# speechcatcher-asr/speechcatcher

Measured on AMD Instinct MI355X. Metric: concurrent real-time streams (audio-seconds/s), de_xl dims, 640 ms (10240-sample) chunk steps, beam 10 CTC+attention, higher is better.
Workload: dtype f32

## Files before the change

### speechcatcher_amd/csrc/common.h

```cpp
#pragma once
#include <hip/hip_runtime.h>
#include <stdint.h>
#include <stdio.h>
#include <math.h>

#include "../../include/scasr.h"

#define SC_LOGZERO (-10000000000.0f)

void sc_set_error(const char *fmt, ...);

const char *sc_hook(const char *name);

#define SC_CHECK_ARG(cond, msg)      \
  do {                               \
    if (!(cond)) {                   \
      sc_set_error("%s: %s", __func__, msg); \
      return SC_ERR_ARG;             \
    }                                \
  } while (0)

#define SC_CHECK_LAUNCH()                                              \
  do {                                                                 \
    hipError_t e__ = hipGetLastError();                                \
    if (e__ != hipSuccess) {                                           \
      sc_set_error("%s: launch failed: %s", __func__, hipGetErrorString(e__)); \
      return SC_ERR_LAUNCH;                                            \
    }                                                                  \
  } while (0)

__host__ __device__ static inline int cdiv(int a, int b) { return (a + b - 1) / b; }

struct ProfScope { bool on; hipEvent_t a, b; hipStream_t st; };
ProfScope sc_prof_begin(hipStream_t st);
void sc_prof_end(ProfScope &p, int kind, double flops, double bytes);

int sc_decode_step_form(const sc_search *sb);
int sc_gemm_colblocks(const float *A, const int32_t *a_rows, int lda, const float *W, const float *bias, float *C,
                      const int32_t *c_rows, int ldc, int M, int N, int K, int ncb, long cb_stride, int flags, void *stream);

int sc_dec_layer_hpw(const sc_search &sb);
int sc_dec_layer_stream_form(const sc_search &sb);
int sc_dec_layer_split_ffn(const sc_search &sb);

int sc_launch_reduce_ln_proj(const float *part, int npart, int part_M, const float *b2, const float *Xin, float *Xout,
                             const int32_t *rows, int M, int D, const float *ln_g, const float *ln_b, float ln_eps,
                             float *XN, const float *Wq, const float *bq, float *Q, int N, hipStream_t st,
                             int by_row = 0, int half_mode = 0);

struct ScHandoff { const int32_t *blkinfo; int R; float *state; int layer; };
int sc_ffn_ln_handoff(const float *XN, int M, int D, int F, const void *W1, const float *b1, const void *W2, const float *b2,
                      float *X, int w_form, const ScHandoff &ho, void *stream);

template <int CTRL>
__device__ __forceinline__ float dpp_mov(float v) {
  return __int_as_float(__builtin_amdgcn_update_dpp(0, __float_as_int(v), CTRL, 0xF, 0xF, true));
}
#define SC_DPP_XOR1 0xB1
#define SC_DPP_XOR2 0x4E
#define SC_DPP_HALF_MIRROR 0x141
#define SC_DPP_ROR4 0x124
#define SC_DPP_ROR8 0x128
#define SC_DPP_ROW_MIRROR 0x140

template <int LPR>
__device__ __forceinline__ float group_sum(float v) {
  v += dpp_mov<SC_DPP_XOR1>(v);
  v += dpp_mov<SC_DPP_XOR2>(v);
  if (LPR >= 8) v += dpp_mov<SC_DPP_HALF_MIRROR>(v);
  if (LPR == 16) v += dpp_mov<SC_DPP_ROW_MIRROR>(v);
  return v;
}

__device__ __forceinline__ float sc_lane(float v, int lane) {
  return __int_as_float(__builtin_amdgcn_readlane(__float_as_int(v), lane));
}
__device__ __forceinline__ float wave_max(float v) {
  v = fmaxf(v, dpp_mov<SC_DPP_XOR1>(v));
  v = fmaxf(v, dpp_mov<SC_DPP_XOR2>(v));
  v = fmaxf(v, dpp_mov<SC_DPP_HALF_MIRROR>(v));
  v = fmaxf(v, dpp_mov<SC_DPP_ROW_MIRROR>(v));
  return fmaxf(fmaxf(sc_lane(v, 0), sc_lane(v, 16)), fmaxf(sc_lane(v, 32), sc_lane(v, 48)));
}
__device__ __forceinline__ float wave_sum(float v) {
  v += dpp_mov<SC_DPP_XOR1>(v);
  v += dpp_mov<SC_DPP_XOR2>(v);
  v += dpp_mov<SC_DPP_HALF_MIRROR>(v);
  v += dpp_mov<SC_DPP_ROW_MIRROR>(v);
  return (sc_lane(v, 0) + sc_lane(v, 16)) + (sc_lane(v, 32) + sc_lane(v, 48));
}
// ... 93 lines not shown
```

### speechcatcher_amd/csrc/search.hip

```cpp
#include "common.h"
#include "attn.h"
#include <mutex>
#include <unordered_map>

#define CTRL(s, f) sb.ctrl[(s) * 8 + (f)]
#define SC_CTC_T(s) (CTRL(s, SC_C_TCTC) > 0 ? CTRL(s, SC_C_TCTC) : CTRL(s, SC_C_T))

#define YSEQ(pp, s, h) (sb.yseq + (((long)(pp) * sb.S + (s)) * sb.W + (h)) * sb.LCAP)
#define XPOS(pp, s, h) (sb.xpos + (((long)(pp) * sb.S + (s)) * sb.W + (h)) * sb.LCAP)
#define ANC(pp, s) (sb.anc + ((long)(pp) * sb.S + (s)) * sb.LCAP * sb.W)
#define CTCR(pp, s) (sb.ctc_r + ((long)(pp) * sb.S + (s)) * sb.TCAP * 2 * sb.W)
#define CTCRS(pp, s) (sb.ctc_rs + ((long)(pp) * sb.S + (s)) * sb.TCAP * sb.W)

__global__ void ctc_extend_state_kernel(sc_search sb) {
  const int s = blockIdx.x, h = threadIdx.x;
  if (!CTRL(s, SC_C_ACTIVE) || !CTRL(s, SC_C_HAS)) return;
  const int T = CTRL(s, SC_C_T), told = CTRL(s, SC_C_TOLD), nh = CTRL(s, SC_C_NHYP);
  if (h >= nh || told >= T) return;
  float *r = CTCR(CTRL(s, SC_C_CUR), s);
  float *rs = CTCRS(CTRL(s, SC_C_CUR), s);
  const float *x = sb.ctcx + (long)s * sb.TCAP * sb.V;
  const int t0 = told < 1 ? 1 : told;
  float rb = r[((long)(t0 - 1) * 2 + 1) * sb.W + h];
  for (int t = t0; t < T; ++t) {
// ... 862 lines not shown
      const bool ok = kw != 0ull && sort_key_value(kw) > bound;
      if (lane == 0) need_full = ok ? 0 : 1;
      if (ok && lane < W) {
        const int i = sort_key_index(key);
        sb.cand_tok[(long)row * W + lane] = i;
        sb.cand_score[(long)row * W + lane] = sort_key_value(key);
        sb.cand_ctc[(long)row * W + lane] = ctc[i];
      }
    }
    __syncthreads();
    if (!need_full) return;
    __syncthreads();
  }
  for (int v = tid; v < V; v += 256) ctc[v] = SC_LOGZERO;
  __syncthreads();
  for (int k = tid; k < K; k += 256) ctc[sb.pre_ids[(long)row * K + k]] = sb.psi[(long)row * K + k];
  __syncthreads();
  if (tid == 0) {
    ctc[sb.eos] = sb.psi_eos[row];
    ctc[sb.blank] = SC_LOGZERO;
  }
  __syncthreads();
  for (int v = tid; v < V; v += 256) {
    const float cv = __fsub_rn(ctc[v], s_prev);
    ctc[v] = cv;
    comb[v] = __fadd_rn(__fmul_rn(sb.w_dec, sb.logp[(long)row * V + v]), __fmul_rn(sb.w_ctc, cv));
  }
  __syncthreads();
  const int NP = next_pow2(V);
  unsigned long long *comp = reinterpret_cast<unsigned long long *>(smem + 2 * V);
  for (int c = tid; c < NP; c += 256) comp[c] = c < V ? sort_key(comb[c], c) : 0ull;
  __syncthreads();
  block_bitonic_sort_desc(comp, NP);
  for (int k = tid; k < W; k += 256) {
    const int i = sort_key_index(comp[k]);
    sb.cand_tok[(long)row * W + k] = i;
    sb.cand_score[(long)row * W + k] = comb[i];
    sb.cand_ctc[(long)row * W + k] = ctc[i];
  }
}

extern "C" int sc_fuse_topw(const sc_search *sbp, void *stream) {
  SC_CHECK_ARG(sbp, "null");
  SC_CHECK_ARG(sbp->V > 0 && sbp->V <= SC_MAX_VOCAB, "vocabulary larger than SC_MAX_VOCAB (8192)");
  const size_t smem = fuse_topw_lds(sbp->V);
  const int rc = allow_large_lds(reinterpret_cast<const void *>(&fuse_topw_kernel), smem, fuse_topw_lds(SC_MAX_VOCAB),
                                 "sc_fuse_topw");
  if (rc != SC_OK) return rc;
  fuse_topw_kernel<<<sbp->S * sbp->W, 256, smem, (hipStream_t)stream>>>(*sbp);
  SC_CHECK_LAUNCH();
  return SC_OK;
}

__global__ __launch_bounds__(256) void beam_prune_kernel(sc_search sb) {
  extern __shared__ __attribute__((aligned(16))) double tot[];
  __shared__ int fl_any, fl_all, fl_best, fl_rep;
  __shared__ int win_h[64], win_tok[64];
  __shared__ unsigned bm[SC_KV_MAX_ROWS / 32];
  const int s = blockIdx.x, tid = threadIdx.x;
  if (!CTRL(s, SC_C_ACTIVE)) return;
  for (int w = tid; w < (sb.kv_rows + 31) / 32; w += 256) bm[w] = 0u;
  const int W = sb.W, K = sb.K;
  const int nh = CTRL(s, SC_C_NHYP), L = CTRL(s, SC_C_L), T = CTRL(s, SC_C_T);
  const int cur = CTRL(s, SC_C_CUR), o = 1 - cur;
  const int n = nh * W, nout = n < W ? n : W;
  if (tid == 0) { fl_any = 0; fl_all = 1; fl_best = 0; fl_rep = 0; }
  for (int e = tid; e < n; e += 256) {
    const int h = e / W, j = e % W;
    tot[e] = sb.score[((long)cur * sb.S + s) * W + h] + (double)sb.cand_score[((long)s * W + h) * W + j];
  }
  __syncthreads();
  for (int e = tid; e < n; e += 256) {
    const double te = tot[e];
    int rk = 0;
    for (int j = 0; j < n; ++j) rk += (tot[j] > te) || (tot[j] == te && j < e);
    if (rk >= nout) continue;
    const int h = e / W, j = e % W, i = rk;
    const long prow = (long)s * W + h;
    const int tok = sb.cand_tok[prow * W + j];
    win_h[i] = h;
    win_tok[i] = tok;
    const long oi = ((long)o * sb.S + s) * W + i, ci = ((long)cur * sb.S + s) * W + h;
    sb.score[oi] = te;
    sb.sc_dec[oi] = sb.sc_dec[ci] + (double)sb.logp[prow * sb.V + tok];
    sb.sc_ctc[oi] = sb.sc_ctc[ci] + (double)sb.cand_ctc[prow * W + j];
    int kk = -1;
    for (int q = 0; q < K; ++q)
      if (sb.pre_ids[prow * K + q] == tok) { kk = q; break; }
    float sval;
    if (tok == sb.blank) sval = SC_LOGZERO;
    else if (tok == sb.eos) sval = sb.psi_eos[prow];
    else if (kk >= 0) sval = sb.psi[prow * K + kk];
    else sval = SC_LOGZERO;
    sb.ctc_s[oi] = sval;
    sb.sel[((long)s * W + i) * 2] = h;
    sb.sel[((long)s * W + i) * 2 + 1] = kk < 0 ? 0 : kk;
    const bool is_eos = tok == sb.eos;
    if (is_eos) atomicOr(&fl_any, 1);
    else atomicAnd(&fl_all, 0);
    if (i == 0 && is_eos) atomicOr(&fl_best, 1);
  }
  __syncthreads();
  const int *asrc = ANC(cur, s);
  int *adst = ANC(o, s);
  bool rep = false;
  constexpr int UB = 4;
  const int ntot = nout * (L + 1);
// ... 9 lines not shown
      av[u] = asrc[(long)p * W + h];
    }
#pragma unroll
    for (int u = 0; u < UB; ++u) {
      const int e = e0 + 256 * u;
      if (e >= ntot) break;
      const int i = e / (L + 1), p = e % (L + 1);
      const int tok = win_tok[i];
      int *ydst = YSEQ(o, s, i), *xdst = XPOS(o, s, i);
      if (p < L) {
        ydst[p] = yv[u];
        xdst[p] = xv[u];
        if (p >= 1 && yv[u] == tok && tok != sb.sos && tok != sb.eos) rep = true;
        adst[(long)p * W + i] = av[u];
        atomicOr(&bm[(av[u] >> 5) & (SC_KV_MAX_ROWS / 32 - 1)], 1u << (av[u] & 31));
      } else {
        ydst[L] = tok;
        xdst[L] = T - 1;
      }
    }
  }
  if (rep) atomicOr(&fl_rep, 1);
  __syncthreads();
  if (tid == 0)
    sb.flags[s] = (fl_any ? SC_F_ANY_EOS : 0) | (fl_best ? SC_F_BEST_EOS : 0) |
                  (fl_all ? SC_F_ALL_EOS : 0) | (fl_rep ? SC_F_REPEAT : 0);
  if (tid >= 64 || L + 1 > sb.LCAP) return;
  const int lane = tid, NR = sb.kv_rows, nwords = (NR + 31) / 32;
  int *out = adst + (long)L * W;
  int got = 0;
  for (int w0 = 0; w0 < nwords && got < nout; w0 += 64) {
    const int w = w0 + lane;
    unsigned fr = w < nwords ? ~bm[w] : 0u;
    if (w == nwords - 1 && (NR & 31)) fr &= (1u << (NR & 31)) - 1u;
    const int c = __popc(fr);
    int incl = c;
#pragma unroll
    for (int o2 = 1; o2 < 64; o2 <<= 1) {
      const int t = __shfl_up(incl, o2, 64);
      if (lane >= o2) incl += t;
    }
    int k = got + incl - c;
    while (fr && k < nout) {
      const int b = __ffs(fr) - 1;
      fr &= fr - 1u;
      out[k++] = w * 32 + b;
    }
    got += __shfl(incl, 63, 64);
  }
  if (got < nout && lane >= got && lane < nout) out[lane] = NR - 1;
  if (lane == 0 && sb.kvflags) sb.kvflags[s] = got < nout ? 1 : 0;
}

extern "C" int sc_beam_prune(const sc_search *sbp, void *stream) {
  SC_CHECK_ARG(sbp, "null");
  SC_CHECK_ARG(sbp->W <= 64, "beam wider than 64");
  SC_CHECK_ARG(sbp->kv_rows >= sbp->W && sbp->kv_rows <= SC_KV_MAX_ROWS, "kv_rows out of range (beam .. 65536)");
  size_t smem = (size_t)sbp->W * sbp->W * sizeof(double);
  beam_prune_kernel<<<sbp->S, 256, smem, (hipStream_t)stream>>>(*sbp);
  SC_CHECK_LAUNCH();
  return SC_OK;
}

__global__ __launch_bounds__(256) void ctc_gather_state_kernel(sc_search sb, int split_min) {
  const int s = blockIdx.y;
  if (!CTRL(s, SC_C_ACTIVE)) return;
  const int W = sb.W, K = sb.K, V = sb.V, T = SC_CTC_T(s), nh = CTRL(s, SC_C_NHYP), L = CTRL(s, SC_C_L);
  const int nout = nh * W < W ? nh * W : W;
  const int cur = CTRL(s, SC_C_CUR), o = 1 - cur;
  const bool has = CTRL(s, SC_C_HAS);
  const int WK = W * K, tct = sb.tct;
  float *dst = CTCR(o, s);
  float *dst_rs = CTCRS(o, s);
  const float *__restrict__ rp = CTCR(cur, s);
  const float *__restrict__ rsp = CTCRS(cur, s);
  const float *ck = sb.ctc_rnew + (long)s * ctc_tck(sb.TCAP) * 2 * WK;
  const int out_len = L - 1;
  int start = out_len > 1 ? out_len : 1;
  if (start > T) start = T;
  const bool split = ctc_scan_is_split(T, L, split_min);
  const int base = start & ~15;
  const int seg = split ? 16 * cdiv(T - base, 16 * CTC_NSEG) : SC_CTC_CK;
  const int nseg = split ? CTC_NSEG : cdiv(T, SC_CTC_CK);
  for (int idx = blockIdx.x * blockDim.x + threadIdx.x; idx < nout * nseg; idx += gridDim.x * blockDim.x) {
    const int i = idx % nout, j = idx / nout;
    const int h = sb.sel[((long)s * W + i) * 2], k = sb.sel[((long)s * W + i) * 2 + 1];
    const int e = h * K + k;
    const int c = sb.pre_ids[((long)s * W + h) * K + k];
    const bool same = c == YSEQ(cur, s, h)[L - 1];
    const float *__restrict__ xcol = sb.ctcxT + ((long)s * V + c) * tct;
    const float *__restrict__ xblk = sb.ctcxT + ((long)s * V + sb.blank) * tct;
    int t_lo, t_hi;
    float r_n, r_b;
    if (split) {
      t_lo = max(start, base + j * seg);
      t_hi = min(T, base + (j + 1) * seg);
      r_n = ck[((long)j * 2) * WK + e];
      r_b = ck[((long)j * 2 + 1) * WK + e];
      if (j == 0) {
        for (int t = 0; t < start - 1; ++t) {
          dst[((long)t * 2) * W + i] = SC_LOGZERO;
          dst[((long)t * 2 + 1) * W + i] = SC_LOGZERO;
          dst_rs[(long)t * W + i] = lse2(SC_LOGZERO, SC_LOGZERO);
        }
        dst[((long)(start - 1) * 2) * W + i] = (out_len == 0) ? xcol[0] : SC_LOGZERO;
        dst[((long)(start - 1) * 2 + 1) * W + i] = SC_LOGZERO;
        dst_rs[(long)(start - 1) * W + i] = lse2((out_len == 0) ? xcol[0] : SC_LOGZERO, SC_LOGZERO);
      }
    } else {
      const int t0 = j * SC_CTC_CK, t1 = min(t0 + SC_CTC_CK, T);
      if (t0 <= start - 1) {
        r_n = (out_len == 0) ? xcol[0] : SC_LOGZERO;
        r_b = SC_LOGZERO;
        for (int t = t0; t < min(start - 1, t1); ++t) {
          dst[((long)t * 2) * W + i] = SC_LOGZERO;
// ... 30 lines not shown
      for (int q = 0; q < SC_CTC_CK; ++q) {
        const int tp = min(max(tb + q - 1, 0), T - 1);
        pn[q] = has ? rsp[(long)tp * W + h] : 0.f;
        pb[q] = has ? rp[((long)tp * 2 + 1) * W + h] : 0.f;
      }
#pragma unroll
      for (int q = 0; q < SC_CTC_CK; ++q) {
        const int t = tb + q;
        if (t >= t_lo && t < t_hi) {
          float phi;
          ctc_frame(r_n, r_b, has ? pn[q] : cum, has ? pb[q] : cum, same, xc[q], xb[q], phi);
          dst[((long)t * 2) * W + i] = r_n;
          dst[((long)t * 2 + 1) * W + i] = r_b;
          dst_rs[(long)t * W + i] = lse2(r_n, r_b);
          if (!has) cum += xb[q];
        }
      }
    }
  }
}

extern "C" int sc_ctc_gather_state_split(const sc_search *sbp, int split_min, void *stream) {
  SC_CHECK_ARG(sbp, "null");
  SC_CHECK_ARG(sbp->ctcxT && sbp->tct >= 4, "the state rebuild needs the column-major table copy (sc_search.ctcxT)");
  int gx = cdiv(ctc_tck(sbp->TCAP) * sbp->W, 256);
  if (gx > 16) gx = 16;
  const int eff = ctc_split_min_ok(sbp->TCAP, split_min), last = scan_split_last(sbp);
  if (last >= 0 && last != eff) {
    sc_set_error("sc_ctc_gather_state_split: the last prefix scan of this batch ran with split_min = %d, the rebuild was asked for %d - "
                 "streams split over T leave segment states, not checkpoints: pass the scan's value (sc_ctc_gather_state() = 0)", last, eff);
    return SC_ERR_ARG;
  }
  ctc_gather_state_kernel<<<dim3(gx, sbp->S), 256, 0, (hipStream_t)stream>>>(*sbp, eff);
  SC_CHECK_LAUNCH();
  return SC_OK;
}

extern "C" int sc_ctc_gather_state(const sc_search *sbp, void *stream) { return sc_ctc_gather_state_split(sbp, 0, stream); }

static bool dec_fused_ok(const sc_search &sb) {
  if (const char *e = sc_hook("SC_DEC_FUSED"))
    return atoi(e) != 0 && sc_dec_layer_fused_supported(sb.d, sb.H, sb.W, sb.F) && sb.ph1 && sb.out_w_q;
  if (const char *e = sc_hook("SC_FUSED_MAX"))
    if ((sb.rowmap ? sb.n_rows : sb.S * sb.W) > atoi(e) && sc_dec_layer_hpw(sb) < 2) return false;
  return sc_dec_layer_fused_supported(sb.d, sb.H, sb.W, sb.F) && sb.ph1 && sb.ph2 && sb.ffn_part &&
         sb.max_ffn_part >= 1 && sb.out_w_q && sb.V % sb.d == 0 && sb.layers && sb.layers[0].wqkv_pp &&
         sb.layers[0].wq_pp && sb.layers[0].wo_pp && sb.layers[0].w1_p;
}

int sc_decode_step_form(const sc_search *sbp) { return dec_fused_ok(*sbp) ? (sc_dec_layer_stream_form(*sbp) ? 2 : 1) : 0; }

extern "C" int sc_decode_step(const sc_search *sbp, void *stream) { return sc_decode_step_ex(sbp, 0, stream); }

extern "C" int sc_decode_step_ex(const sc_search *sbp, int scan_split_min, void *stream) {
  SC_CHECK_ARG(sbp, "null");
  const sc_search &sb = *sbp;
  const int n = sb.rowmap ? sb.n_rows : sb.S * sb.W;
  int rc;
  if (dec_fused_ok(sb) && sc_dec_layer_stream_form(sb)) {
    float *xa = sb.dx, *xb = sb.dxn;
    int npart = 0;
    for (int li = 0; li < sb.n_layers; ++li) {
      SC_TRY(sc_dec_layer_stream(sbp, li, xa, xb, sb.dq, sb.ffn_part, npart, stream));
      SC_TRY(sc_dec_layer_ffn_xn(sbp, li, sb.dq, sb.ffn_part, sb.max_ffn_part, &npart, stream));
      float *t = xa; xa = xb; xb = t;
    }
    SC_TRY(sc_dec_output_logits(sbp, xa, xb, sb.ffn_part, npart, stream));
  } else if (dec_fused_ok(sb)) {
    float *xa = sb.dx, *xb = sb.dxn;
    int npart = 0;
    for (int li = 0; li < sb.n_layers; ++li) {
      SC_TRY(sc_dec_layer_self(sbp, li, xa, xb, sb.ffn_part, npart, stream));
      SC_TRY(sc_dec_layer_cross(sbp, li, xb, xa, stream));
      if (sc_dec_layer_split_ffn(sb)) {
        SC_TRY(sc_dec_layer_reduce_ln(sbp, li, xa, xb, sb.dq, stream));
        SC_TRY(sc_dec_layer_ffn_xn(sbp, li, sb.dq, sb.ffn_part, sb.max_ffn_part, &npart, stream));
      } else
      SC_TRY(sc_dec_layer_ffn(sbp, li, xa, xb, sb.ffn_part, sb.max_ffn_part, &npart, stream));
      float *t = xa; xa = xb; xb = t;
    }
    SC_TRY(sc_dec_output_logits(sbp, xa, xb, sb.ffn_part, npart, stream));
  } else {
  SC_TRY(sc_dec_embed(sbp, stream));
  bool logits_done = false;
  SC_TRY(decoder_layers_impl(sbp, stream, true, &logits_done));
  if (!logits_done)
    SC_TRY(sc_gemm(sb.dxn, sb.rowmap, sb.d, sb.out_w, sb.out_b, sb.logits, sb.rowmap, sb.V, n, sb.V, sb.d, 0, 0, stream));
  }
  SC_TRY(sc_logsoftmax_topk(sbp, stream));
  const bool use_ctc = sb.w_ctc > 0.f;
  if (use_ctc) SC_TRY(sc_ctc_prefix_scan_split(sbp, scan_split_min, stream));
  SC_TRY(sc_fuse_topw(sbp, stream));
  SC_TRY(sc_beam_prune(sbp, stream));
  if (use_ctc) SC_TRY(sc_ctc_gather_state_split(sbp, scan_split_min, stream));
  return SC_OK;
}
```

### speechcatcher_amd/csrc/streams.hip

```cpp
#include <algorithm>
#include <array>
#include <chrono>
#include <cmath>
#include <cstdarg>
#include <cstring>
#include <deque>
#include <map>
#include <memory>
#include <new>
#include <string>
#include <vector>

#include "common.h"

namespace {

#define HIP_TRY(call)                                                              \
  do {                                                                             \
    hipError_t e__ = (call);                                                       \
    if (e__ != hipSuccess) {                                                       \
      sc_set_error("%s: %s failed: %s", __func__, #call, hipGetErrorString(e__));  \
      return SC_ERR_LAUNCH;                                                        \
    }                                                                              \
  } while (0)
#define RC_TRY(call)                 \
  do {                               \
    int rc__ = (call);               \
    if (rc__ != SC_OK) return rc__;  \
  } while (0)

struct Tensor {
  void *ptr = nullptr;
  int64_t numel = 0;
  int dtype = 0;
  bool owned = false;
};

struct StreamFault {
  int stream;
  int code;
  std::string msg;
};

}

struct sc_engine {
  sc_config cfg{};
  int device = 0;
  std::map<std::string, Tensor> t;
  std::vector<sc_enc_layer> enc;
  std::vector<sc_dec_layer> dec;
  std::vector<const float *> wkv, bkv;
  float *wkv_all = nullptr, *bkv_all = nullptr;

  const float *f(const std::string &name, bool required = true) const {
    auto it = t.find(name);
    if (it == t.end()) {
      if (required) sc_set_error("sc_engine: tensor '%s' is missing", name.c_str());
      return nullptr;
    }
    return (const float *)it->second.ptr;
  }
  ~sc_engine() {
    for (auto &kv : t)
      if (kv.second.owned && kv.second.ptr) (void)hipFree(kv.second.ptr);
    if (wkv_all) (void)hipFree(wkv_all);
// ... 49 lines not shown
};

template <typename T>
int dalloc(T **p, size_t n) {
  const size_t bytes = std::max<size_t>(n, 1) * sizeof(T);
  HIP_TRY(hipMalloc((void **)p, bytes));
  HIP_TRY(hipMemset(*p, 0, bytes));
  return SC_OK;
}

}

struct EncPlan {
  std::vector<int32_t> conv_jobs, a_rows, lin_dst, feat_src, feat_dst, blk_jobs, sjobs, emit_src, emit_dst, sub_src,
      sub_dst;
  struct Short { int s, ubase, U, pe_pos, dst_T; };
  std::vector<Short> shorts;
  int n_conv = 0, max_t1 = 0;
};

struct EncGroup {
  long gen = 0;
  bool launched = false, features = false;
  bool open = false;
  bool deferred = false;
  int slot = 0;
  int stage_slot = -1;
  std::vector<long long> copy_jobs;
  size_t stage_floats = 0;
  std::vector<int32_t> fe_jobs;
  int n_fe = 0, max_keep = 0;
  EncPlan P;
  std::vector<int32_t> ctc_rows, kv_src, kv_dst;
  bool same_rows = true;
  std::vector<int> streams;
  bool empty() const { return !n_fe && !P.n_conv; }
};

constexpr int N_ARENA = 8;
constexpr int N_STAGE = 4;
constexpr int N_RING = 4;

struct sc_streams {
  sc_engine *eng = nullptr;
  sc_config cfg{};
  int S = 0, W = 0, K = 0, TCAP = 0, LCAP = 0, FCAP = 0, UCAP = 0, max_feat_new = 0, max_t1 = 0, max_t2 = 0,
      max_blocks = 0, max_chunk = 0, max_length = 500;
  long PCAP = 0;
  bool use_bbd = false, strict = true;
  hipStream_t stream = nullptr;
  hipStream_t stream_enc = nullptr, es = nullptr;
  hipEvent_t ev_iter[2] = {nullptr, nullptr};
  int32_t *ring_dev = nullptr;
  int32_t *rm_host[2] = {nullptr, nullptr};
  int rm_idx = 0;
  bool rm_dirty = false;
  int scan_split_min = 1024, scan_split_streams = 0;
  bool scan_long = false;
  int step_split_min() const { return (scan_long && (scan_split_streams <= 0 || n_rows_step <= scan_split_streams * W)) ? scan_split_min : 0; }
  int graph_key() const { return n_rows_step * 2 + (step_split_min() > 0 ? 1 : 0); }
  int enc_start_thr = 0;
  int enc_batch_min = 0;
  int gemm_flags = 0;
  void *ws = nullptr, *ws_enc = nullptr;
  std::vector<void *> owned, owned_host;
  float *pcm = nullptr, *featbuf = nullptr, *subbuf = nullptr, *prev_addin = nullptr, *past_ctx = nullptr, *enc = nullptr,
        *c1 = nullptr, *c2 = nullptr, *xblk = nullptr, *ws_xn = nullptr, *ws_qkv = nullptr, *ws_att = nullptr,
        *ws_ffh = nullptr;
  int32_t *jobs_ctx = nullptr, *ctrlmap = nullptr;
  float *kv_stage = nullptr;
  int kv_stage_rows = 0;
  sc_search sb{};
  int32_t *ctrlmap_host = nullptr, *flags_host = nullptr;
  int32_t *arena_host = nullptr, *arena_dev = nullptr;
  size_t slot_cap = 0, arena_off = 0;
  int cur_slot = 0;
  hipEvent_t ev_group[N_ARENA] = {nullptr};
  long slot_gen[N_ARENA] = {0};
  int32_t *bs_host = nullptr, *bs_dev = nullptr;
  size_t bs_cap = 0;
  int bs_i = 0;
  float *stage_host = nullptr, *stage_dev = nullptr;
  size_t stage_cap = 0;
  hipEvent_t ev_stage[N_STAGE] = {nullptr};
  bool stage_busy[N_STAGE] = {false};
  int stage_next = 0;
  long long *cjobs_host = nullptr, *cjobs_dev = nullptr;
  int32_t *pack_dev = nullptr, *pack_host = nullptr, *pjobs_host = nullptr, *pjobs_dev = nullptr;
  size_t pack_cap = 0;
  char *al_dev = nullptr;
  size_t al_cap = 0;
  std::vector<St> st;
  std::vector<Run> run;
  std::vector<std::deque<Blk>> bq;
  std::vector<Job> job;
  std::vector<std::deque<Job>> ahead;
  std::vector<long> job_seq;
  int queue_depth = 1;
  std::vector<Snap> snap;
  std::vector<long> done_at;
  long done_counter = 0;
  int32_t *snap_yseq = nullptr, *snap_xpos = nullptr;
  double *snap_score = nullptr;
  hipEvent_t ev_snap = nullptr;
  std::vector<std::string> fault_msg;
  std::vector<long> enc_gen;
// ... 419 lines not shown
    std::vector<int32_t> j_add(ns * 4), j_ctx(ns * 4);
    for (int i = 0; i < ns; ++i) {
      const int32_t *sj = &P.sjobs[i * 5];
      j_add[i * 4 + 0] = sj[0]; j_add[i * 4 + 1] = sj[1]; j_add[i * 4 + 2] = sj[2]; j_add[i * 4 + 3] = sj[3];
      j_ctx[i * 4 + 0] = sj[0]; j_ctx[i * 4 + 1] = sj[1]; j_ctx[i * 4 + 2] = sj[2] * c.enc_layers; j_ctx[i * 4 + 3] = sj[4];
    }
    RC_TRY(b->itensor(j_add, &ja));
    RC_TRY(sc_ctx_handoff(b->xblk, R, ja, ns, b->prev_addin, 0, d, b->es));
    const int32_t *jc;
    RC_TRY(b->itensor(j_ctx, &jc));
    HIP_TRY(hipMemcpyAsync(b->jobs_ctx, jc, j_ctx.size() * sizeof(int32_t), hipMemcpyDeviceToDevice, b->es));
    RC_TRY(enc_layers_launch(b, nbk, R, true, b->jobs_ctx, ns));
  }
  if (!P.emit_src.empty()) {
    const int32_t *a, *z;
    RC_TRY(b->itensor(P.emit_src, &a));
    RC_TRY(b->itensor(P.emit_dst, &z));
    RC_TRY(sc_layernorm(b->xblk, a, d, b->enc, z, d, (int)P.emit_src.size(), d, e->f("enc_norm_g"), e->f("enc_norm_b"),
                        c.ln_eps, b->es));
  }
  for (auto &sh : P.shorts) RC_TRY(encode_short(b, sh));
  if (!P.sub_src.empty()) {
    const int32_t *a, *z;
    RC_TRY(b->itensor(P.sub_src, &a));
    RC_TRY(b->itensor(P.sub_dst, &z));
    RC_TRY(sc_copy_rows(b->subbuf, a, b->subbuf, z, (int)P.sub_src.size(), d, b->es));
  }
  return SC_OK;
}

void set_rowmap(sc_streams *b, const std::vector<int> &active) {
  const int S = b->S, W = b->W;
  const int na = (int)active.size();
  const int nb = std::min(S, (na + b->row_bucket - 1) / b->row_bucket * b->row_bucket);
  if (active != b->rowmap_key) {
    b->rowmap_key = active;
    b->rm_idx ^= 1;
    b->rm_dirty = true;
    int32_t *rm = b->rowmap_host();
    std::vector<char> isact(S, 0);
    for (int s : active) isact[s] = 1;
    int k = 0;
    for (int pass = 1; pass >= 0; --pass)
      for (int s = 0; s < S; ++s)
        if (isact[s] == pass)
          for (int h = 0; h < W; ++h) rm[k++] = s * W + h;
  }
  b->n_rows_step = nb * W;
}

int decode_step_launch(sc_streams *b) {
  b->sb.n_rows = b->n_rows_step;
  b->sb.flags = b->ring_dev;
  auto step = [&]() { return sc_decode_step_ex(&b->sb, b->step_split_min(), b->stream); };
  if (!b->use_graphs) return step();
  auto it = b->dec_graphs.find(b->graph_key());
  if (it == b->dec_graphs.end()) {
    RC_TRY(step());
    RC_TRY(sc_graph_capture_begin(b->stream));
    const int rc = step();
    void *g = nullptr;
    const int rc2 = sc_graph_capture_end(b->stream, &g);
    if (rc != SC_OK) return rc;
    if (rc2 != SC_OK) return rc2;
    b->dec_graphs[b->graph_key()] = (hipGraphExec_t)g;
    return SC_OK;
  }
  return sc_graph_launch(it->second, b->stream);
}

int prepare_decode(sc_streams *b) {
  memset(b->ctrl_host(), 0, (size_t)b->S * 8 * sizeof(int32_t));
  HIP_TRY(hipMemcpyAsync(b->ctrlmap, b->ctrlmap_host, (size_t)b->S * 8 * sizeof(int32_t), hipMemcpyHostToDevice, b->stream));
  const int keep = b->n_rows_step;
  for (int nb = b->row_bucket; nb < b->S + b->row_bucket; nb += b->row_bucket) {
    b->n_rows_step = std::min(nb, b->S) * b->W;
    if (!b->dec_graphs.count(b->graph_key())) RC_TRY(decode_step_launch(b));
  }
  b->n_rows_step = keep;
  HIP_TRY(hipStreamSynchronize(b->stream));
  return SC_OK;
}

int retire_groups(sc_streams *b) {
  while (!b->groups.empty()) {
    EncGroup *g = b->groups.front();
    if (!g->launched) break;
    const hipError_t q = hipEventQuery(b->ev_group[g->slot]);
    if (q == hipErrorNotReady) { (void)hipGetLastError(); break; }
    if (q != hipSuccess) {
      sc_set_error("encoder group %ld failed: %s", g->gen, hipGetErrorString(q));
      return SC_ERR_LAUNCH;
    }
    b->gen_done = g->gen;
    b->slot_gen[g->slot] = 0;
    b->groups.pop_front();
    delete g;
  }
  return SC_OK;
}

int launch_pending_groups(sc_streams *b, long upto = -1);
int wait_group(sc_streams *b, long gen) {
  if (gen <= b->gen_done) return SC_OK;
  RC_TRY(launch_pending_groups(b, gen));
  const int slot = (int)(gen % N_ARENA);
  HIP_TRY(hipEventSynchronize(b->ev_group[slot]));
  return retire_groups(b);
}

int project_rows(sc_streams *b, EncGroup &g) {
  const sc_config &c = b->cfg;
  sc_engine *e = b->eng;
  const int d = c.d_model, Ld = c.dec_layers, V = c.vocab_size;
  const int32_t *ar = nullptr;
  if (!g.ctc_rows.empty()) {
    RC_TRY(b->itensor(g.ctc_rows, &ar));
    RC_TRY(sc_gemm(b->enc, ar, d, e->f("ctc_w"), e->f("ctc_b"), const_cast<float *>(b->sb.ctcx), ar, V, (int)g.ctc_rows.size(),
                   V, d, b->gemm_flags, 0, b->es));
  }
  if (!g.kv_dst.empty()) {
    if (!g.same_rows || !ar) RC_TRY(b->itensor(g.kv_src, &ar));
    const int32_t *kvt;
    RC_TRY(b->itensor(g.kv_dst, &kvt));
    const int m = (int)g.kv_dst.size();
    const bool all = e->wkv_all && (2 * d) % 128 == 0;
// ... 238 lines not shown
    long upto = -1;
    for (EncGroup *g : b->groups)
      if (!g->launched && g->deferred && g->gen <= need) upto = g->gen;
    if (upto >= 0) RC_TRY(launch_pending_groups(b, upto));
  }
  std::vector<int> &active = b->tick_active;
  active.clear();
  for (int s = 0; s < S; ++s) {
    Run &r = b->run[s];
    if (!r.inblk) continue;
    const bool act = r.live && r.pidx < b->max_length;
    if (act && r.L + 1 > b->LCAP) {
      fault_stream(b, s, SC_ERR_CAPACITY, "max_tokens exceeded");
      *progress = true;
      continue;
    }
    if (!act) {
      finish_block(b, s);
      *progress = true;
      continue;
    }
    active.push_back(s);
  }
  if (active.empty()) {
    if (*progress) return SC_OK;
    long need = 0;
    for (int s = 0; s < S; ++s)
      if (!b->run[s].inblk && !b->bq[s].empty() && (need == 0 || b->bq[s].front().gen < need)) need = b->bq[s].front().gen;
    if (need > std::max(b->gen_done, b->gen_ordered)) {
      RC_TRY(launch_pending_groups(b, need));
      if (b->stream_enc) HIP_TRY(hipStreamWaitEvent(b->stream, b->ev_group[need % N_ARENA], 0));
      b->gen_ordered = std::max(b->gen_ordered, need);
      *progress = true;
    }
    return SC_OK;
  }
  *progress = true;
  b->tick_t0 = std::chrono::steady_clock::now();
  set_rowmap(b, active);
  b->scan_long = false;
  int32_t *ctrl = b->ctrl_host();
  memset(ctrl, 0, (size_t)S * 8 * sizeof(int32_t));
  for (int s : active) {
    const Run &r = b->run[s];
    if (b->scan_split_min > 0 && r.Tc - std::max(r.L - 1, 1) >= b->scan_split_min) b->scan_long = true;
    int32_t *c = ctrl + s * 8;
    c[0] = 1; c[1] = r.cur; c[2] = r.fin; c[3] = r.T; c[4] = r.L; c[5] = r.nhyp; c[6] = r.has; c[7] = r.Tc;
  }
  if ((int)active.size() <= b->enc_start_thr)
    for (EncGroup *g : b->groups)
      if (!g->launched && !g->open) RC_TRY(launch_group(b, g));
  if (b->rm_dirty) {
    memcpy(b->ctrlmap_host + S * 8, b->rm_host[b->rm_idx], (size_t)S * W * sizeof(int32_t));
    HIP_TRY(hipMemcpyAsync(b->ctrlmap, b->ctrlmap_host, (size_t)(S * 8 + S * W) * sizeof(int32_t), hipMemcpyHostToDevice, b->stream));
    b->rm_dirty = false;
  } else {
    HIP_TRY(hipMemcpyAsync(b->ctrlmap, b->ctrlmap_host, (size_t)S * 8 * sizeof(int32_t), hipMemcpyHostToDevice, b->stream));
  }
  RC_TRY(decode_step_launch(b));
  HIP_TRY(hipEventRecord(b->ev_iter[b->iter & 1], b->stream));
  const int form = sc_decode_step_form(&b->sb);
  for (int s : active) {
    b->xattn_rows[form] += (long)b->run[s].T * Ld;
    b->sattn_pos[form] += (long)b->run[s].L * Ld;
  }
  b->tick_t1 = std::chrono::steady_clock::now();
  b->inflight = true;
  return SC_OK;
}

int tick_collect(sc_streams *b) {
  if (!b->inflight) return SC_OK;
  const int S = b->S, W = b->W;
  b->inflight = false;
  const auto tpw = std::chrono::steady_clock::now();
  HIP_TRY(hipEventSynchronize(b->ev_iter[b->iter & 1]));
  const auto tp2 = std::chrono::steady_clock::now();
  b->iter++;
  b->dec_steps++;
  b->t_launch += std::chrono::duration<double>(b->tick_t1 - b->tick_t0).count();
  b->t_wait += std::chrono::duration<double>(tp2 - tpw).count();
  {
    const int bk = std::min(16, (int)((long)b->n_rows_step * 16 / std::max(1, S * W)));
    b->t_bucket[bk] += std::chrono::duration<double>(tp2 - b->tick_t0).count();
    b->n_bucket[bk] += 1;
  }
  for (int s : b->tick_active) {
    Run &r = b->run[s];
    const bool kv_full = b->flags_host[S + s] != 0;
    b->flags_host[S + s] = 0;
    const int f = b->flags_host[s];
    const bool f_any = f & F_ANY_EOS, f_best = f & F_BEST_EOS, f_all = f & F_ALL_EOS, f_rep = f & F_REPEAT;
    r.out += 1;
    r.nsteps += 1;
    const bool stop_eos = f_any && (!r.fin || f_best);
    const bool stop_bbd = b->use_bbd && !stop_eos && f_rep && !r.fin;
    const bool stop_all = !stop_eos && !stop_bbd && f_all && r.fin;
    const bool accept = !(stop_eos || stop_bbd || stop_all);
    const bool take = stop_eos || stop_all || accept;
    if (kv_full && take && !(!accept && r.pidx > 1 && r.pvalid)) {
      if (sc_hook("SC_DEBUG_POOL"))
        fprintf(stderr, "[scasr] pool exhausted: stream %d L %d nhyp %d T %d fin %d pidx %d flags %d kv_rows %d iter %ld\n", s, r.L, r.nhyp,
                r.T, (int)r.fin, r.pidx, f, b->sb.kv_rows, b->iter);
      fault_stream(b, s, SC_ERR_CAPACITY, "self-attention K|V pool exhausted (kv_pool_rows / max_tokens)");
      continue;
    }
    if (stop_bbd) r.out -= 1;
    if (take) {
      r.nhp = r.nhyp;
      r.hasp = r.has;
      r.cur = 1 - r.cur;
      r.L += 1;
      r.nhyp = std::min(W, r.nhyp * W);
      r.has = true;
    }
    if (stop_eos || stop_all) r.took = true;
    r.live = accept;
    if (accept) {
      r.pvalid = true;
      r.pidx += 1;
    }
    if (!(r.live && r.pidx < b->max_length)) finish_block(b, s);
  }
  return SC_OK;
}

int engine_tick(sc_streams *b, bool *progress) {
  RC_TRY(tick_issue(b, progress));
  return tick_collect(b);
// ... 546 lines not shown
  }
  if (rc == SC_OK && hipMalloc(&b->ws, (size_t)128 << 20) != hipSuccess) rc = SC_ERR_LAUNCH;
  if (rc == SC_OK) b->owned.push_back(b->ws);
#undef A
  if (rc != SC_OK) {
    sc_set_error("sc_streams_create: device allocation failed");
    delete b;
    return rc;
  }
  sb.ctrl = b->ctrlmap;
  sb.rowmap = b->ctrlmap + S * 8;
  sb.n_rows = S * W;
  sb.embed = e->f("embed"); sb.pe = e->f("pe"); sb.dec_norm_g = e->f("dec_norm_g"); sb.dec_norm_b = e->f("dec_norm_b");
  sb.out_w = e->f("out_w"); sb.out_b = e->f("out_b"); sb.out_w_q = e->f("out_w_q", false);
  sb.out_w_qh = nullptr;
  sb.act_half = 0;
  if (sb.kv_half && e->f("out_w_qh", false) && !e->dec.empty() && e->dec[0].wqkv_pph && e->dec[0].wq_pph && e->dec[0].wo_pph &&
      e->dec[0].wo2_pph && sb.ph1) {
    sb.out_w_qh = e->f("out_w_qh", false);
    sb.act_half = 1 | 2;
    if (const char *ah = sc_hook("SC_ACT_HALF")) sb.act_half = atoi(ah) & 7;
  }
  sb.layers = e->dec.data();
  (void)sc_set_stream_workspace(b->stream, b->ws, (size_t)128 << 20);
  b->es = b->stream;
  {
    const char *th = sc_hook("SC_ENC_START");
    b->enc_start_thr = S < 16 ? S : std::max(1, (int)((long)S * (th ? atoi(th) : 7) / 100));
  }
  {
    const char *ov = sc_hook("SC_ENC_OVERLAP");
    if (!(ov && atoi(ov) == 0)) {
      const char *cu = sc_hook("SC_ENC_CUS");
      const int ncu = cu ? atoi(cu) : 0;
      hipError_t er;
      if (ncu > 0 && ncu < 256) {
        uint32_t mask[8] = {0, 0, 0, 0, 0, 0, 0, 0};
        for (int i = 0; i < ncu; ++i) mask[i >> 5] |= 1u << (i & 31);
        er = hipExtStreamCreateWithCUMask(&b->stream_enc, 8, mask);
      } else {
        er = hipStreamCreateWithPriority(&b->stream_enc, hipStreamNonBlocking, sc_hook("SC_PRIO_ENC") ? atoi(sc_hook("SC_PRIO_ENC")) : 0);
      }
      if (er == hipSuccess && hipMalloc(&b->ws_enc, (size_t)128 << 20) == hipSuccess) {
        b->owned.push_back(b->ws_enc);
        (void)sc_set_stream_workspace(b->stream_enc, b->ws_enc, (size_t)128 << 20);
      } else {
        (void)hipGetLastError();
        if (b->stream_enc) (void)hipStreamDestroy(b->stream_enc);
        b->stream_enc = nullptr;
      }
    }
  }
  const size_t cm = ((size_t)S * 8 + n) * sizeof(int32_t);
  bool ok = b->halloc(&b->ctrlmap_host, (size_t)S * 8 + n) == SC_OK && b->halloc(&b->flags_host, (size_t)S * 2) == SC_OK &&
            b->halloc(&b->rm_host[0], n) == SC_OK && b->halloc(&b->rm_host[1], n) == SC_OK &&
            b->halloc(&b->arena_host, b->slot_cap * N_ARENA) == SC_OK && b->halloc(&b->bs_host, b->bs_cap * N_RING) == SC_OK &&
            b->halloc(&b->stage_host, b->stage_cap * N_STAGE) == SC_OK && b->halloc(&b->pack_host, b->pack_cap) == SC_OK &&
            b->halloc(&b->pjobs_host, n * 4) == SC_OK && b->halloc(&b->cjobs_host, (size_t)N_STAGE * S * 3) == SC_OK;
  for (int i = 0; i < 2 && ok; ++i) ok = hipEventCreateWithFlags(&b->ev_iter[i], hipEventDisableTiming) == hipSuccess;
  for (int i = 0; i < N_ARENA && ok; ++i) ok = hipEventCreateWithFlags(&b->ev_group[i], hipEventDisableTiming) == hipSuccess;
  for (int i = 0; i < N_STAGE && ok; ++i) ok = hipEventCreateWithFlags(&b->ev_stage[i], hipEventDisableTiming) == hipSuccess;
  if (!ok) {
    sc_set_error("sc_streams_create: pinned host allocation failed");
    delete b;
    return SC_ERR_LAUNCH;
  }
  memset(b->flags_host, 0, (size_t)S * 8);
  {
    void *dv = nullptr;
    if (hipHostGetDevicePointer(&dv, b->flags_host, 0) != hipSuccess || !dv) {
      sc_set_error("sc_streams_create: pinned flags are not device-accessible");
      delete b;
      return SC_ERR_LAUNCH;
    }
    b->ring_dev = (int32_t *)dv;
    sb.flags = b->ring_dev;
    sb.kvflags = b->ring_dev + S;
  }
  if (const char *sp = sc_hook("SC_SCAN_SPLIT_MIN")) b->scan_split_min = atoi(sp);
  if (const char *sp = sc_hook("SC_SCAN_SPLIT_STREAMS")) b->scan_split_streams = atoi(sp);
  memset(b->ctrlmap_host, 0, cm);
  for (size_t i = 0; i < n; ++i) b->rm_host[0][i] = b->rm_host[1][i] = (int32_t)i;
  (void)hipMemcpy(b->ctrlmap, b->ctrlmap_host, (size_t)S * 8 * sizeof(int32_t), hipMemcpyHostToDevice);
  (void)hipMemcpy(b->ctrlmap + S * 8, b->rm_host[0], n * sizeof(int32_t), hipMemcpyHostToDevice);
  b->rowmap_key.resize(S);
  for (int s = 0; s < S; ++s) b->rowmap_key[s] = s;
  b->enc_batch_min = std::max(1, S / 2);
  b->gemm_flags = (!b->eng->enc.empty() && b->eng->enc[0].wqkv_s) ? SC_GEMM_SPLIT16 : 0;
  b->row_bucket = std::max(1, S / 32);
  if (const char *rb = sc_hook("SC_ROW_BUCKETS")) b->row_bucket = std::max(1, S / std::max(1, atoi(rb)));
  b->n_rows_step = S * W;
  b->st.assign(S, St());
  b->run.assign(S, Run());
  b->bq.assign(S, std::deque<Blk>());
  b->job.assign(S, Job());
  b->ahead.assign(S, std::deque<Job>());
  b->job_seq.assign(S, 0);
  b->snap.assign(S, Snap());
  b->done_at.assign(S, 0);
  b->fault_msg.assign(S, std::string());
  b->enc_gen.assign(S, 0);
  for (int s = 0; s < S; ++s) init_hyp(b, s);
  *out = b;
  return SC_OK;
  SC_API_END
}

extern "C" void sc_streams_destroy(sc_streams *b) {
  if (b) {
    (void)hipStreamSynchronize(b->stream);
    if (b->stream_enc) (void)hipStreamSynchronize(b->stream_enc);
    delete b;
  }
}

extern "C" int sc_reset(sc_streams *b, int stream) {
  SC_CHECK_ARG(b && stream >= 0 && stream < b->S, "stream out of range");
  SC_CHECK_ARG(!b->job[stream].open, "the stream has a chunk outstanding (sc_poll reports it first)");
  reset_stream(b, stream);
  return SC_OK;
}

extern "C" void *sc_streams_hip_stream(sc_streams *b) { return b ? (void *)b->stream : nullptr; }

extern "C" float *sc_streams_pcm(sc_streams *b, long *capacity) {
  if (!b) return nullptr;
  if (capacity) *capacity = b->PCAP;
  return b->pcm;
}

namespace {

int report_chunk(sc_streams *b, int s) {
  Job &j = b->job[s];
  const int status = j.fault ? j.fault : j.has_out;
// ... 571 lines not shown
```

Measured before the change: 4070.

## Stage control map via device kernel and signal step completion through pinned publish word

Replaces the per-step host-to-device memcpy of the control map and row map with a small kernel that reads the pinned host image directly over system-scope loads into device memory. The beam prune kernel now counts finished blocks and, in the last one, sets a pinned publish word. The host spins on that word, polling the event occasionally, instead of calling hipEventSynchronize. This aims to cut copy-engine round trips and the wake-up latency of the blocking event wait, so the CPU can read the beam results earlier. The cost is host CPU spinning. It also risks returning before the trailing gather kernel finishes and races if the host rewrites the pinned ctrl image while the staging kernel reads it.

```diff
diff --git a/speechcatcher_amd/csrc/common.h b/speechcatcher_amd/csrc/common.h
--- a/speechcatcher_amd/csrc/common.h
+++ b/speechcatcher_amd/csrc/common.h
@@ -36,6 +36,8 @@
 void sc_prof_end(ProfScope &p, int kind, double flops, double bytes);
 
 int sc_decode_step_form(const sc_search *sb);
+int sc_decode_step_handoff(const sc_search *sbp, int scan_split_min, const int32_t *ctrl_src, int32_t *ctrl_dst, int n_ctrl,
+                           int32_t *pub_cnt, int32_t *pub_word, void *stream);
 int sc_gemm_colblocks(const float *A, const int32_t *a_rows, int lda, const float *W, const float *bias, float *C,
                       const int32_t *c_rows, int ldc, int M, int N, int K, int ncb, long cb_stride, int flags, void *stream);
 
diff --git a/speechcatcher_amd/csrc/host_wait.h b/speechcatcher_amd/csrc/host_wait.h
--- /dev/null
+++ b/speechcatcher_amd/csrc/host_wait.h
@@ -0,0 +1,37 @@
+#pragma once
+#include <chrono>
+#include <cstdint>
+
+namespace sc_host_wait {
+
+enum Result {
+  SEEN = 0,
+  EVENT_DONE = 1,
+  BUDGET = 2,
+  FAILED = -1,
+};
+
+template <class Query>
+Result wait_word(const volatile int32_t *word, Query &&query, double query_every_us, double budget_us) {
+  using clk = std::chrono::steady_clock;
+  const auto t0 = clk::now();
+  const auto every = std::chrono::duration<double, std::micro>(query_every_us);
+  const auto budget = std::chrono::duration<double, std::micro>(budget_us);
+  auto next = t0 + every;
+  for (;;) {
+    if (__atomic_load_n(word, __ATOMIC_ACQUIRE) != 0) return SEEN;
+    const auto now = clk::now();
+    if (now >= next) {
+      const int q = query();
+      if (q < 0) return FAILED;
+      if (q == 0) return __atomic_load_n(word, __ATOMIC_ACQUIRE) != 0 ? SEEN : EVENT_DONE;
+      if (now - t0 >= budget) return BUDGET;
+      next = now + every;
+    }
+#if defined(__x86_64__) || defined(__i386__)
+    __builtin_ia32_pause();
+#endif
+  }
+}
+
+}
diff --git a/speechcatcher_amd/csrc/search.hip b/speechcatcher_amd/csrc/search.hip
--- a/speechcatcher_amd/csrc/search.hip
+++ b/speechcatcher_amd/csrc/search.hip
@@ -938,7 +938,7 @@
   return SC_OK;
 }
 
-__global__ __launch_bounds__(256) void beam_prune_kernel(sc_search sb) {
+__device__ __forceinline__ void beam_prune_body(const sc_search &sb) {
   extern __shared__ __attribute__((aligned(16))) double tot[];
   __shared__ int fl_any, fl_all, fl_best, fl_rep;
   __shared__ int win_h[64], win_tok[64];
@@ -1054,15 +1054,34 @@
   if (lane == 0 && sb.kvflags) sb.kvflags[s] = got < nout ? 1 : 0;
 }
 
-extern "C" int sc_beam_prune(const sc_search *sbp, void *stream) {
+__device__ __forceinline__ void step_publish(int32_t *pub_cnt, int32_t *pub_word) {
+  __threadfence();
+  __syncthreads();
+  if (threadIdx.x == 0) {
+    const int n = (int)(gridDim.x * gridDim.y * gridDim.z);
+    if (__hip_atomic_fetch_add(pub_cnt, 1, __ATOMIC_ACQ_REL, __HIP_MEMORY_SCOPE_SYSTEM) == n - 1) {
+      __hip_atomic_store(pub_cnt, 0, __ATOMIC_RELAXED, __HIP_MEMORY_SCOPE_AGENT);
+      __hip_atomic_store(pub_word, 1, __ATOMIC_RELEASE, __HIP_MEMORY_SCOPE_SYSTEM);
+    }
+  }
+}
+
+__global__ __launch_bounds__(256) void beam_prune_kernel(sc_search sb, int32_t *pub_cnt, int32_t *pub_word) {
+  beam_prune_body(sb);
+  if (pub_word) step_publish(pub_cnt, pub_word);
+}
+
+static int beam_prune_launch(const sc_search *sbp, int32_t *pub_cnt, int32_t *pub_word, void *stream) {
   SC_CHECK_ARG(sbp, "null");
   SC_CHECK_ARG(sbp->W <= 64, "beam wider than 64");
   SC_CHECK_ARG(sbp->kv_rows >= sbp->W && sbp->kv_rows <= SC_KV_MAX_ROWS, "kv_rows out of range (beam .. 65536)");
   size_t smem = (size_t)sbp->W * sbp->W * sizeof(double);
-  beam_prune_kernel<<<sbp->S, 256, smem, (hipStream_t)stream>>>(*sbp);
+  beam_prune_kernel<<<sbp->S, 256, smem, (hipStream_t)stream>>>(*sbp, pub_cnt, pub_word);
   SC_CHECK_LAUNCH();
   return SC_OK;
 }
+
+extern "C" int sc_beam_prune(const sc_search *sbp, void *stream) { return beam_prune_launch(sbp, nullptr, nullptr, stream); }
 
 __global__ __launch_bounds__(256) void ctc_gather_state_kernel(sc_search sb, int split_min) {
   const int s = blockIdx.y;
@@ -1199,9 +1218,25 @@
 
 extern "C" int sc_decode_step(const sc_search *sbp, void *stream) { return sc_decode_step_ex(sbp, 0, stream); }
 
+__global__ __launch_bounds__(256) void ctrl_stage_kernel(const int32_t *src, int32_t *dst, int n) {
+  for (int i = blockIdx.x * blockDim.x + threadIdx.x; i < n; i += gridDim.x * blockDim.x)
+    dst[i] = __hip_atomic_load(src + i, __ATOMIC_RELAXED, __HIP_MEMORY_SCOPE_SYSTEM);
+}
+
 extern "C" int sc_decode_step_ex(const sc_search *sbp, int scan_split_min, void *stream) {
+  return sc_decode_step_handoff(sbp, scan_split_min, nullptr, nullptr, 0, nullptr, nullptr, stream);
+}
+
+int sc_decode_step_handoff(const sc_search *sbp, int scan_split_min, const int32_t *ctrl_src, int32_t *ctrl_dst, int n_ctrl,
+                           int32_t *pub_cnt, int32_t *pub_word, void *stream) {
   SC_CHECK_ARG(sbp, "null");
+  SC_CHECK_ARG(!ctrl_src || (ctrl_dst && n_ctrl > 0), "ctrl staging needs a destination and a size");
+  SC_CHECK_ARG(!pub_word || pub_cnt, "the publish word needs its counter");
   const sc_search &sb = *sbp;
+  if (ctrl_src) {
+    ctrl_stage_kernel<<<cdiv(n_ctrl, 256) < 8 ? cdiv(n_ctrl, 256) : 8, 256, 0, (hipStream_t)stream>>>(ctrl_src, ctrl_dst, n_ctrl);
+    SC_CHECK_LAUNCH();
+  }
   const int n = sb.rowmap ? sb.n_rows : sb.S * sb.W;
   int rc;
   if (dec_fused_ok(sb) && sc_dec_layer_stream_form(sb)) {
@@ -1238,7 +1273,7 @@
   const bool use_ctc = sb.w_ctc > 0.f;
   if (use_ctc) SC_TRY(sc_ctc_prefix_scan_split(sbp, scan_split_min, stream));
   SC_TRY(sc_fuse_topw(sbp, stream));
-  SC_TRY(sc_beam_prune(sbp, stream));
+  SC_TRY(beam_prune_launch(sbp, pub_cnt, pub_word, stream));
   if (use_ctc) SC_TRY(sc_ctc_gather_state_split(sbp, scan_split_min, stream));
   return SC_OK;
 }
diff --git a/speechcatcher_amd/csrc/streams.hip b/speechcatcher_amd/csrc/streams.hip
--- a/speechcatcher_amd/csrc/streams.hip
+++ b/speechcatcher_amd/csrc/streams.hip
@@ -12,6 +12,7 @@
 #include <vector>
 
 #include "common.h"
+#include "host_wait.h"
 
 namespace {
 
@@ -167,6 +168,8 @@
   hipStream_t stream_enc = nullptr, es = nullptr;
   hipEvent_t ev_iter[2] = {nullptr, nullptr};
   int32_t *ring_dev = nullptr;
+  int32_t *pub_host = nullptr, *pub_dev = nullptr, *pub_cnt = nullptr;
+  const int32_t *ctrl_src = nullptr;
   int32_t *rm_host[2] = {nullptr, nullptr};
   int rm_idx = 0;
   bool rm_dirty = false;
@@ -692,7 +695,10 @@
 int decode_step_launch(sc_streams *b) {
   b->sb.n_rows = b->n_rows_step;
   b->sb.flags = b->ring_dev;
-  auto step = [&]() { return sc_decode_step_ex(&b->sb, b->step_split_min(), b->stream); };
+  auto step = [&]() {
+    return sc_decode_step_handoff(&b->sb, b->step_split_min(), b->ctrl_src, b->ctrlmap, b->S * 8 + b->S * b->W, b->pub_cnt,
+                                  b->pub_dev, b->stream);
+  };
   if (!b->use_graphs) return step();
   auto it = b->dec_graphs.find(b->graph_key());
   if (it == b->dec_graphs.end()) {
@@ -711,7 +717,6 @@
 
 int prepare_decode(sc_streams *b) {
   memset(b->ctrl_host(), 0, (size_t)b->S * 8 * sizeof(int32_t));
-  HIP_TRY(hipMemcpyAsync(b->ctrlmap, b->ctrlmap_host, (size_t)b->S * 8 * sizeof(int32_t), hipMemcpyHostToDevice, b->stream));
   const int keep = b->n_rows_step;
   for (int nb = b->row_bucket; nb < b->S + b->row_bucket; nb += b->row_bucket) {
     b->n_rows_step = std::min(nb, b->S) * b->W;
@@ -1056,11 +1061,9 @@
       if (!g->launched && !g->open) RC_TRY(launch_group(b, g));
   if (b->rm_dirty) {
     memcpy(b->ctrlmap_host + S * 8, b->rm_host[b->rm_idx], (size_t)S * W * sizeof(int32_t));
-    HIP_TRY(hipMemcpyAsync(b->ctrlmap, b->ctrlmap_host, (size_t)(S * 8 + S * W) * sizeof(int32_t), hipMemcpyHostToDevice, b->stream));
     b->rm_dirty = false;
-  } else {
-    HIP_TRY(hipMemcpyAsync(b->ctrlmap, b->ctrlmap_host, (size_t)S * 8 * sizeof(int32_t), hipMemcpyHostToDevice, b->stream));
-  }
+  }
+  __atomic_store_n(b->pub_host, 0, __ATOMIC_RELAXED);
   RC_TRY(decode_step_launch(b));
   HIP_TRY(hipEventRecord(b->ev_iter[b->iter & 1], b->stream));
   const int form = sc_decode_step_form(&b->sb);
@@ -1073,12 +1076,37 @@
   return SC_OK;
 }
 
+int wait_step(sc_streams *b) {
+  hipEvent_t ev = b->ev_iter[b->iter & 1];
+  hipError_t err = hipSuccess;
+  auto query = [&]() {
+    const hipError_t q = hipEventQuery(ev);
+    if (q == hipSuccess) return 0;
+    if (q == hipErrorNotReady) {
+      (void)hipGetLastError();
+      return 1;
+    }
+    err = q;
+    return -1;
+  };
+  switch (sc_host_wait::wait_word(b->pub_host, query, 20.0, 50000.0)) {
+    case sc_host_wait::SEEN:
+    case sc_host_wait::EVENT_DONE: return SC_OK;
+    case sc_host_wait::FAILED:
+      sc_set_error("decode step failed: %s", hipGetErrorString(err));
+      return SC_ERR_LAUNCH;
+    case sc_host_wait::BUDGET: break;
+  }
+  HIP_TRY(hipEventSynchronize(ev));
+  return SC_OK;
+}
+
 int tick_collect(sc_streams *b) {
   if (!b->inflight) return SC_OK;
   const int S = b->S, W = b->W;
   b->inflight = false;
   const auto tpw = std::chrono::steady_clock::now();
-  HIP_TRY(hipEventSynchronize(b->ev_iter[b->iter & 1]));
+  RC_TRY(wait_step(b));
   const auto tp2 = std::chrono::steady_clock::now();
   b->iter++;
   b->dec_steps++;
@@ -1731,7 +1759,7 @@
     }
   }
   const size_t cm = ((size_t)S * 8 + n) * sizeof(int32_t);
-  bool ok = b->halloc(&b->ctrlmap_host, (size_t)S * 8 + n) == SC_OK && b->halloc(&b->flags_host, (size_t)S * 2) == SC_OK &&
+  bool ok = b->halloc(&b->ctrlmap_host, (size_t)S * 8 + n) == SC_OK && b->halloc(&b->flags_host, (size_t)S * 2 + 1) == SC_OK &&
             b->halloc(&b->rm_host[0], n) == SC_OK && b->halloc(&b->rm_host[1], n) == SC_OK &&
             b->halloc(&b->arena_host, b->slot_cap * N_ARENA) == SC_OK && b->halloc(&b->bs_host, b->bs_cap * N_RING) == SC_OK &&
             b->halloc(&b->stage_host, b->stage_cap * N_STAGE) == SC_OK && b->halloc(&b->pack_host, b->pack_cap) == SC_OK &&
@@ -1755,11 +1783,20 @@
     b->ring_dev = (int32_t *)dv;
     sb.flags = b->ring_dev;
     sb.kvflags = b->ring_dev + S;
+    b->pub_host = b->flags_host + 2 * S;
+    b->pub_dev = b->ring_dev + 2 * S;
+    void *cv = nullptr;
+    if (hipHostGetDevicePointer(&cv, b->ctrlmap_host, 0) != hipSuccess || !cv || b->alloc(&b->pub_cnt, 1) != SC_OK) {
+      sc_set_error("sc_streams_create: pinned ctrl image is not device-accessible");
+      delete b;
+      return SC_ERR_LAUNCH;
+    }
+    b->ctrl_src = (const int32_t *)cv;
   }
   if (const char *sp = sc_hook("SC_SCAN_SPLIT_MIN")) b->scan_split_min = atoi(sp);
   if (const char *sp = sc_hook("SC_SCAN_SPLIT_STREAMS")) b->scan_split_streams = atoi(sp);
   memset(b->ctrlmap_host, 0, cm);
-  for (size_t i = 0; i < n; ++i) b->rm_host[0][i] = b->rm_host[1][i] = (int32_t)i;
+  for (size_t i = 0; i < n; ++i) b->rm_host[0][i] = b->rm_host[1][i] = b->ctrlmap_host[S * 8 + i] = (int32_t)i;
   (void)hipMemcpy(b->ctrlmap, b->ctrlmap_host, (size_t)S * 8 * sizeof(int32_t), hipMemcpyHostToDevice);
   (void)hipMemcpy(b->ctrlmap + S * 8, b->rm_host[0], n * sizeof(int32_t), hipMemcpyHostToDevice);
   b->rowmap_key.resize(S);
```

Result: no change. 3995, median of 2 (-1.8%).
